# wonheeML/mtl-ssl

Hardware: AMD Instinct MI355X
Metric: images/sec training, Faster R-CNN ResNet-101 + aux heads (higher is better)
Workload: dtype f32; 1 GPU; Faster R-CNN ResNet-101 + window/closeness/edgemask heads + refine, synthetic 1024x600 COCO-shaped (90 classes), per-GPU batch 2 (BASELINE.json configs[1]); global_batch=2, parallelism=dp1, pipeline_config=configs/frcnn_resnet101_coco_mtl.config

## Files before the change

### mtl_ssl_amd/csrc/conv.hip

```cpp
#include <stdlib.h>

#include <atomic>
#include <mutex>
#include <unordered_map>

#include "conv_mfma.h"
#include "conv_split.h"

namespace mtlssl {

__global__ void __launch_bounds__(256) k_row_group_flags(const float* __restrict__ scale, int n, uint8_t* __restrict__ flags) {
  const int i = blockIdx.x * blockDim.x + threadIdx.x;
  if (i < n) flags[i] = scale[i] != 0.f;
}
__global__ void __launch_bounds__(256) k_active_ksteps(const uint8_t* __restrict__ flags, int rpg, int P, int pps, int stride,
                                                       int* __restrict__ out) {
  const int z = blockIdx.x, pix0 = z * pps, pix1 = min(P, pix0 + pps);
  const int ksteps = (max(pix1 - pix0, 0) + BK - 1) / BK;
  const int lane = threadIdx.x & 63, w = threadIdx.x >> 6;
  int* list = out + KSTEP_HDR + (int64_t)z * stride;
  __shared__ int wave_cnt[4];
  int base = 0;
  for (int s0 = 0; s0 < ksteps; s0 += 256) {
    const int s = s0 + threadIdx.x;
// ... 1421 lines not shown
  MTLSSL_REQUIRE(!group_active || rows_per_group > 0, "conv_dgrad: group_active needs rows_per_group > 0");
  MTLSSL_REQUIRE(!(epi & MASK_ANY) || mask_ref, "conv_dgrad: mask_ref pointer required");
  MTLSSL_REQUIRE(!(epi & MTLSSL_EPI_RESIDUAL) || residual, "conv_dgrad: residual pointer required");
  ConvArgs p = make_args(d);
  p.a = dy; p.b = w; p.out = dx; p.residual = residual; p.mask = mask_ref; p.epi = epi;
  p.a_bytes = ydy_bytes(d);
  p.b_bytes = (unsigned)((int64_t)d->R * d->S * d->C * d->K * 4);
  p.M = d->N * d->H * d->W;
  p.NG = d->C;
  MTLSSL_REQUIRE(desc_dense(d) || mfma_dgrad_ok(d),
                 "conv_dgrad: a strided dy (ldy = %d) needs K %% 16 == 0, C %% 4 == 0 and C >= 16", d->ldy);
  const Route r = route(d, MODE_DGRAD, workspace != nullptr);
  switch (r.family) {
    case FAM_WINO:
      wino_dgrad(d, r.wc.variant, r.wc.tile, dy, w, residual, mask_ref, dx, epi, workspace, S(stream),
                 (filter_xf && xf_variant == r.wc.variant) ? filter_xf : nullptr);
      break;
    case FAM_PARITY:
      parity_dgrad(r, d, dy, w, residual, mask_ref, dx, epi, workspace, S(stream));
      break;
    case FAM_DIRECT:
      if (group_active && row_skip_ref().load() != 0 && desc_is_pointwise(d)) {
        p.group_active = group_active;
        p.rows_per_group = rows_per_group;
      }
      launch_planned<MODE_DGRAD>(r.plan, p, (float*)workspace, S(stream));
      break;
    case FAM_PADDED: {
      float* dy_pad = (float*)workspace;
      float* w_pad = (float*)((char*)workspace + r.front_a);
      hipLaunchKernelGGL(k_pad_rows, dim3(cdiv((int64_t)p.M * r.q.K, 256)), dim3(256), 0, S(stream), dy, (int64_t)p.M, d->K, r.q.K, dy_pad);
// ... 108 lines not shown
  if (int rc = check_desc(d)) return rc;
  static const int32_t PUBLIC[] = {MTLSSL_PLAN_WINO_F43, MTLSSL_PLAN_DIRECT, MTLSSL_PLAN_PARITY, MTLSSL_PLAN_PADDED, MTLSSL_PLAN_S2D,
                                   MTLSSL_PLAN_THIN,     MTLSSL_PLAN_VALU,   MTLSSL_PLAN_VALU,   MTLSSL_PLAN_VALU,   MTLSSL_PLAN_VALU};
  const Route r = route(d, mode);
  const mtlssl_conv_desc& q = r.q;
  for (int i = 0; i < MTLSSL_PLAN_INFO_LEN; ++i) out[i] = 0;
  out[0] = PUBLIC[r.family];
  out[1] = mtlssl_conv2d_tile_config(d, mode);
  out[2] = -1;
  out[14] = mtlssl_conv2d_num_dispatches(d, mode);
  const int64_t P = (int64_t)d->N * d->OH * d->OW, M = mode == MODE_FWD ? P : (int64_t)d->N * d->H * d->W;
  switch (r.family) {
    case FAM_WINO:
      if (r.wc.variant != 0) out[0] = MTLSSL_PLAN_WINO_M7;
      out[2] = r.wc.tile; out[3] = 1;
      out[9] = (int32_t)(mode == MODE_WGRAD ? d->C : M);
      out[10] = mode == MODE_DGRAD ? d->C : d->K;
      out[11] = CFG_BM[r.wc.tile]; out[12] = CFG_BN[r.wc.tile];
      break;
    case FAM_PARITY: {
      MTLSSL_REQUIRE(parity_class >= 0 && parity_class < 4, "plan_info: parity class %d of an input-parity dgrad", parity_class);
      const ParityProblem c = parity_problem(d, parity_class >> 1, parity_class & 1);
      if (c.Hs == 0 || c.Ws == 0 || c.Rs == 0 || c.Ss == 0) break;
      const Plan& pl = r.parity[parity_class];
      plan_info_gemm(pl, (int64_t)d->N * c.Hs * c.Ws, d->C, c.Rs * c.Ss * (d->K / CFG_BK[pl.cfg]), out);
      break;
    }
    case FAM_DIRECT: case FAM_PADDED: case FAM_S2D:
      if (mode == MODE_WGRAD) {
        const int cfg = r.wg.cfg;
// ... 103 lines not shown
  bool colsum_folded = false;
  auto colsum_partial = [&]() {
    const int kg = (int)cdiv(d->K, (d->K & 3) ? 1 : 4);
    dim3 grid(cdiv(kg, cp.CQ), cp.chunks);
    if (d->K & 3)
      hipLaunchKernelGGL(k_colsum_partial<float>, grid, dim3(256), 0, st, dy, (int)P, d->K, ldy, cp.per_chunk, cp.CQ,
                         (float*)workspace);
    else
      hipLaunchKernelGGL(k_colsum_partial<floatx4>, grid, dim3(256), 0, st, dy, (int)P, d->K, ldy, cp.per_chunk, cp.CQ,
                         (float*)workspace);
  };
  const Route r = route(d, MODE_WGRAD);
  switch (r.family) {
    case FAM_WINO:
      wino_wgrad(d, r.wc.variant, r.wc.tile, x, dy, out_scale, dw, beta, ws_main, st,
                 (input_xf && input_variant == r.wc.variant) ? input_xf : nullptr);
      break;
    case FAM_DIRECT: {
      const bool split = wgrad_on_split_engine(r, d);
      const int ns = split ? r.split_ns : r.wg.nsplit, pps = split ? r.split_pps : r.wg.pps;
      const bool ride = dbias && !split && ns <= COLSUM_MAX_PARTS;
      if (dbias && !ride) colsum_partial();
      p.out = ws_main;
      p.M = d->C; p.NG = d->K; p.nsplit = ns; p.pix_per_split = pps;
      p.cs_part = ride ? (float*)workspace : nullptr;
      if (group_active && row_skip_ref().load() != 0 && !split && desc_is_pointwise(d) && pointwise_ref().load() != 0 &&
          ns <= KSTEP_HDR) {
        int* list = (int*)((char*)ws_main + r.bytes);
        const int stride = (int)cdiv(pps, BK);
        hipLaunchKernelGGL(k_active_ksteps, dim3(ns), dim3(256), 0, st, group_active, rows_per_group, (int)P, pps, stride, list);
        p.k_steps = list;
// ... 60 lines not shown
```

### mtl_ssl_amd/csrc/conv_mfma.h

```cpp
#pragma once
#include <type_traits>

#include "common.h"

namespace mtlssl {

typedef float floatx16 __attribute__((ext_vector_type(16)));
typedef float floatx4 __attribute__((ext_vector_type(4)));

enum { MODE_FWD = 0, MODE_DGRAD = 1, MODE_WGRAD = 2 };
__device__ __forceinline__ float act_mask(float g, float y, int epi) {
  bool on = y > 0.f && (!(epi & MTLSSL_EPI_MASK6) || y < 6.f);
  return on ? g : 0.f;
}
constexpr int MASK_ANY = MTLSSL_EPI_MASK | MTLSSL_EPI_MASK6;
constexpr int BK = 16;
#ifndef MTLSSL_LAB_FLAGS
#define MTLSSL_LAB_FLAGS 0
#endif
constexpr int LAB = MTLSSL_LAB_FLAGS;

struct ConvArgs {
  const float* a;
  const float* b;
// ... 184 lines not shown
  constexpr bool B_KC = (MODE == MODE_DGRAD);
  constexpr int A_LD = BM / RP, B_LD = BN / RP;
  constexpr unsigned OOB = 0xFFFFFFF0u;
  constexpr int LDT = 36;
  constexpr int SMEM_OPS = 2 * BKT * (LDA + LDB), SMEM_EPI = NW * 32 * LDT;
  __shared__ __attribute__((aligned(16))) float smem[SMEM_OPS > SMEM_EPI ? SMEM_OPS : SMEM_EPI];
  float* const sA = smem;
  float* const sB = smem + 2 * BKT * LDA;

  int nwg = p.tiles_m * p.tiles_n;
  int bid = blockIdx.x;
  {
    int q = nwg / 8, r = nwg % 8, xcd = bid % 8, loc = bid / 8;
    bid = (xcd < r ? xcd * (q + 1) : r * (q + 1) + (xcd - r) * q) + loc;
  }
  const int tile_m = bid / p.tiles_n + p.tile_m0, tile_n = bid % p.tiles_n;
  const int m0 = tile_m * BM, n0 = tile_n * BN;
  const int tid = threadIdx.x, lane = tid & 63, wid = tid >> 6;
  const int wr = wid >> 1, wc = wid & 1;
  const int lo = lane & 31, hi = lane >> 5;
  const int kq4 = (tid % KQ) * 4;

  if constexpr (BATCH) {
    p.a += (int64_t)blockIdx.y * p.a_bs;
    p.b += (int64_t)blockIdx.y * p.b_bs;
    if constexpr (MODE != MODE_WGRAD) p.out += (int64_t)blockIdx.y * p.o_bs;
  }
  if constexpr (MODE == MODE_WGRAD && !BATCH) {
    if (p.a_tab) {
      const int grp = blockIdx.z / p.nsplit;
// ... 3 lines not shown
  }
  const int ldy = args_ldy(p);
  int rs_fixed = 0, pix0 = 0, pix1 = 0, ksteps, ks_begin = 0;
  const int* steps = nullptr;
  if constexpr (MODE == MODE_FWD) {
    ksteps = p.R * p.S * (p.C / BKT);
  } else if constexpr (MODE == MODE_DGRAD) {
    ksteps = p.R * p.S * (p.K / BKT);
  } else {
    rs_fixed = BATCH ? 0 : blockIdx.y;
    int split = (!BATCH && p.a_tab) ? blockIdx.z % p.nsplit : blockIdx.z;
    int P = p.N * p.OH * p.OW;
    pix0 = split * p.pix_per_split;
    pix1 = min(P, pix0 + p.pix_per_split);
    ksteps = (max(pix1 - pix0, 0) + BKT - 1) / BKT;
    if constexpr (PW && !BATCH)
      if (p.k_steps) {
        steps = p.k_steps + KSTEP_HDR + split * p.k_stride;
        ksteps = p.k_steps[split];
      }
  }
  unsigned a_rec = p.a_bytes, b_rec = p.b_bytes;
  if constexpr (PW && MODE == MODE_WGRAD) {
    a_rec = min(a_rec, (unsigned)(max(pix1, 0) * p.C) * 4u);
    b_rec = min(b_rec, (unsigned)(max(pix1, 0) * ldy) * 4u);
  }
  __amdgpu_buffer_rsrc_t rsrc_a = __builtin_amdgcn_make_buffer_rsrc(const_cast<float*>(p.a), 0, a_rec, 0x00020000);
  __amdgpu_buffer_rsrc_t rsrc_b = __builtin_amdgcn_make_buffer_rsrc(const_cast<float*>(p.b), 0, b_rec, 0x00020000);
  if constexpr (MODE != MODE_WGRAD) {
    if (p.nsplit > 1) {
      ks_begin = blockIdx.z * p.ks_per_split;
      ksteps = min(ksteps, ks_begin + p.ks_per_split);
    }
  }
  if constexpr (PW && MODE == MODE_DGRAD && !SEG && !BATCH)
    if (p.group_active && !tile_rows_active(p, m0, BM)) ksteps = ks_begin;

  int a_base[A_LD], a_y[A_LD], a_x[A_LD], a_n[A_LD];
  bool a_ok[A_LD];
  unsigned a_voff[A_LD];
  unsigned b_base[B_LD];
  if constexpr (PW && MODE == MODE_WGRAD) {
#pragma unroll
    for (int i = 0; i < A_LD; ++i) {
      const int u = tid + NT * i;
      const int col = m0 + (u % (BM / 4)) * 4;
      a_voff[i] = col < p.M ? (unsigned)((pix0 + u / (BM / 4)) * p.C + col) * 4u : OOB;
    }
  } else if constexpr (PW) {
#pragma unroll
    for (int i = 0; i < A_LD; ++i) {
// ... 348 lines not shown
  constexpr int STAGE = A_FL + B_FL;
  constexpr int PA = BM * BKT / 256 / NW, PB = BN * BKT / 256 / NW;
  constexpr int G = BKT / 8;
  constexpr unsigned OOB = 0xFFFFFFF0u;
  constexpr int LDT = 36;
  constexpr int SMEM_OPS = NSTAGE * STAGE, SMEM_EPI = NW * 32 * LDT;
  __shared__ __attribute__((aligned(16))) float smem[SMEM_OPS > SMEM_EPI ? SMEM_OPS : SMEM_EPI];
  typedef __attribute__((address_space(3))) void* lds_ptr_t;

  int nwg = p.tiles_m * p.tiles_n;
  int bid = blockIdx.x;
  {
    int q = nwg / 8, r = nwg % 8, xcd = bid % 8, loc = bid / 8;
    bid = (xcd < r ? xcd * (q + 1) : r * (q + 1) + (xcd - r) * q) + loc;
  }
  const int tile_m = bid / p.tiles_n + p.tile_m0, tile_n = bid % p.tiles_n;
  const int m0 = tile_m * BM, n0 = tile_n * BN;
  const int tid = threadIdx.x, lane = tid & 63, wid = tid >> 6;
  const int wr = wid >> 1, wc = wid & 1;
  const int lo = lane & 31, hi = lane >> 5;
  auto kc_row = [&](int piece) { return piece * RPP + lane / QPR; };
  auto kc_quad4 = [&](int row) { return (((lane % QPR) ^ ((row >> RSH) & (QPR - 1)))) * 4; };

  if constexpr (BATCH) {
    p.a += (int64_t)blockIdx.y * p.a_bs;
    p.b += (int64_t)blockIdx.y * p.b_bs;
    if constexpr (MODE != MODE_WGRAD) p.out += (int64_t)blockIdx.y * p.o_bs;
  }
  int rs_fixed = 0, pix0 = 0, pix1 = 0, ksteps, ks_begin = 0;
  const int* steps = nullptr;
  if constexpr (MODE == MODE_FWD) {
    ksteps = p.R * p.S * (p.C / BKT);
  } else if constexpr (MODE == MODE_DGRAD) {
    ksteps = p.R * p.S * (p.K / BKT);
  } else {
    rs_fixed = BATCH ? 0 : blockIdx.y;
    int split = blockIdx.z;
    int P = p.N * p.OH * p.OW;
    pix0 = split * p.pix_per_split;
    pix1 = min(P, pix0 + p.pix_per_split);
    ksteps = (max(pix1 - pix0, 0) + BKT - 1) / BKT;
    if constexpr (PWISE && !BATCH)
      if (p.k_steps) {
        steps = p.k_steps + KSTEP_HDR + split * p.k_stride;
        ksteps = p.k_steps[split];
      }
  }
  if constexpr (MODE != MODE_WGRAD) {
    if (p.nsplit > 1) {
      ks_begin = blockIdx.z * p.ks_per_split;
      ksteps = min(ksteps, ks_begin + p.ks_per_split);
    }
  }
  if constexpr (PWISE && MODE == MODE_DGRAD && !BATCH)
    if (p.group_active && !tile_rows_active(p, m0, BM)) ksteps = ks_begin;

  const int ldy = args_ldy(p);
  unsigned a_rec = p.a_bytes, b_rec = p.b_bytes;
  if constexpr (PWISE && MODE == MODE_WGRAD) {
    a_rec = min(a_rec, (unsigned)(max(pix1, 0) * p.C) * 4u);
    b_rec = min(b_rec, (unsigned)(max(pix1, 0) * ldy) * 4u);
  }
  const __amdgpu_buffer_rsrc_t rsrc_a = __builtin_amdgcn_make_buffer_rsrc(const_cast<float*>(p.a), 0, a_rec, 0x00020000);
  const __amdgpu_buffer_rsrc_t rsrc_b = __builtin_amdgcn_make_buffer_rsrc(const_cast<float*>(p.b), 0, b_rec, 0x00020000);

  int a_base[PA], a_y[PA], a_x[PA], a_n[PA], a_q4[PA];
  bool a_ok[PA];
  unsigned a_voff[PA];
  unsigned b_base[PB];
  if constexpr (PWISE && MODE == MODE_WGRAD) {
// ... 381 lines not shown
  double occ_eff = occ <= 1 ? 0.55 : (occ == 2 ? 0.80 : 1.0);
  double step_us = CFG_BM[cfg] * CFG_BN[cfg] * 2.0 * CFG_BK[cfg] / 614e9 * 1e6 / (base_eff[cfg & 3] * occ_eff);
  return (double)per_cu * (ksteps_per_block + 96 / CFG_BK[cfg]) * step_us;
}

enum { WINO_F43 = 0, WINO_M7 = 1, WINO_VARIANTS = 2 };
bool wino_eligible(const mtlssl_conv_desc* d, int variant);
double wino_time_us(const mtlssl_conv_desc* d, int variant, int mode, int* tile);
int64_t wino_workspace_bytes(const mtlssl_conv_desc* d, int variant, int mode);
void wino_fwd(const mtlssl_conv_desc* d, int variant, int tile, const float* x, const float* w, const float* bias,
              const float* residual, float* y, int epi, void* workspace, hipStream_t st, const float* filter_xf = nullptr,
              float* input_xf_keep = nullptr);
int64_t wino_input_bytes(const mtlssl_conv_desc* d, int variant);
void wino_dgrad(const mtlssl_conv_desc* d, int variant, int tile, const float* dy, const float* w,
                const float* residual, const float* mask_ref, float* dx, int epi, void* workspace, hipStream_t st,
                const float* filter_xf = nullptr);
int64_t wino_filter_bytes(const mtlssl_conv_desc* d, int variant);
void wino_filter(const mtlssl_conv_desc* d, int variant, int flip, const float* w, float* U, hipStream_t st);
void wino_filters_batched(int variant, int n, const void* w_ptrs, const void* u_ptrs, const int64_t* ck,
                          const int32_t* flip, int64_t max_ck, hipStream_t st);
void wino_wgrad(const mtlssl_conv_desc* d, int variant, int tile, const float* x, const float* dy,
                const float* out_scale, float* dw, float beta, void* workspace, hipStream_t st,
                const float* input_xf = nullptr);

}
```

### mtl_ssl_amd/csrc/winograd.hip

```cpp
#include "conv_mfma.h"
#include "conv_split.h"

namespace mtlssl {

namespace {

struct F43 {
  static constexpr int P = 6, I = 6, O = 4;
  static constexpr float bt(int a, int i) {
    constexpr float t[6][6] = {{4, 0, -5, 0, 1, 0}, {0, -4, -4, 1, 1, 0}, {0, 4, -4, -1, 1, 0},
                               {0, -2, -1, 2, 1, 0}, {0, 2, -1, -2, 1, 0}, {0, 4, 0, -5, 0, 1}};
    return t[a][i];
  }
  static constexpr float at(int u, int a) {
    constexpr float t[4][6] = {{1, 1, 1, 1, 1, 0}, {0, 1, -1, 2, -2, 0}, {0, 1, 1, 4, 4, 0}, {0, 1, -1, 8, -8, 1}};
    return t[u][a];
  }
  static constexpr float g(int a, int r) {
    constexpr float t[6][3] = {{1.f / 4, 0, 0}, {-1.f / 6, -1.f / 6, -1.f / 6}, {-1.f / 6, 1.f / 6, -1.f / 6},
                               {1.f / 24, 1.f / 12, 1.f / 6}, {1.f / 24, -1.f / 12, 1.f / 6}, {0, 0, 1}};
    return t[a][r];
  }
};
struct F33 {
// ... 41 lines not shown
        if (first) acc = (c == 1.f) ? d[i] : c * d[i];
        else if (c == 1.f) acc = acc + d[i];
        else if (c == -1.f) acc = acc - d[i];
        else acc = acc + c * d[i];
        first = false;
      }
    }
    o[a] = acc;
  }
}

struct WinoGeom {
  int N, H, W, th, tw;
  int64_t T;
};
struct TileIdx { int64_t t; int c, n, ty, tx; bool ok; };
template <typename VT>
__device__ __forceinline__ TileIdx tile_index(const WinoGeom& g, int C) {
  constexpr int VW = sizeof(VT) / 4;
  TileIdx r;
  const int cq = C / VW;
  int64_t idx = blockIdx.x * (int64_t)256 + threadIdx.x;
  r.ok = idx < g.T * cq;
  r.c = (int)(idx % cq) * VW;
  r.t = idx / cq;
  r.tx = (int)(r.t % g.tw);
  int64_t q = r.t / g.tw;
  r.ty = (int)(q % g.th);
  r.n = (int)(q / g.th);
  return r;
}
__device__ __forceinline__ float act_fwd(float v, int epi) {
  if (epi & MTLSSL_EPI_RELU) v = fmaxf(v, 0.f);
  if (epi & MTLSSL_EPI_RELU6) v = fminf(fmaxf(v, 0.f), 6.f);
  if (epi & MTLSSL_EPI_TANH) v = tanhf(v);
  return v;
}
__device__ __forceinline__ floatx4 act_fwd(floatx4 v, int epi) {
#pragma unroll
  for (int q = 0; q < 4; ++q) v[q] = act_fwd(v[q], epi);
  return v;
}
// ... 33 lines not shown
  int64_t i = (blockIdx.x * (int64_t)256 + threadIdx.x) * (sizeof(VT) / 4);
  if (i >= CK) return;
  wino_filter_one<S, VT>(w, U, CK, flip, i);
}
template <typename S>
__global__ void __launch_bounds__(256) k_wino_filter_batched(const float* const* w, float* const* U, const int64_t* CK,
                                                             const int32_t* flip) {
  const int l = blockIdx.y;
  const int64_t ck = CK[l];
  int64_t i = blockIdx.x * (int64_t)256 + threadIdx.x;
  if (i >= ck) return;
  wino_filter_one<S, float>(w[l], U[l], ck, flip[l], i);
}

template <typename S, typename VT>
__global__ void __launch_bounds__(256) k_wino_input(const float* in, float* V, WinoGeom g, int C, int ld) {
  constexpr int P = S::P, I = S::I;
  const TileIdx ix = tile_index<VT>(g, C);
  if (!ix.ok) return;
  const int y0 = S::O * ix.ty - 1, x0 = S::O * ix.tx - 1;
  const float* base = in + ((int64_t)ix.n * g.H * g.W) * ld + ix.c;
  VT tmp[P][I];
#pragma unroll
  for (int j = 0; j < I; ++j) {
    const int x = x0 + j;
    const bool okx = (unsigned)x < (unsigned)g.W;
    VT col[I], o[P];
#pragma unroll
    for (int i = 0; i < I; ++i) {
      const int y = y0 + i;
      const bool ok = okx && (unsigned)y < (unsigned)g.H;
      col[i] = ok ? *reinterpret_cast<const VT*>(base + ((int64_t)y * g.W + x) * ld) : VT{};
    }
    xform<S, XF_BT, P, I>(col, o);
#pragma unroll
    for (int a = 0; a < P; ++a) tmp[a][j] = o[a];
  }
  const int64_t plane = g.T * C;
  float* vp = V + ix.t * C + ix.c;
#pragma unroll
  for (int a = 0; a < P; ++a) {
    VT o[P];
    xform<S, XF_BT, P, I>(tmp[a], o);
#pragma unroll
    for (int b = 0; b < P; ++b) *reinterpret_cast<VT*>(vp + (int64_t)(a * P + b) * plane) = o[b];
  }
}

template <typename S, typename VT>
__global__ void __launch_bounds__(256) k_wino_dy(const float* dy, float* dM, WinoGeom g, int K, int ld) {
  constexpr int P = S::P, O = S::O;
  const TileIdx ix = tile_index<VT>(g, K);
  if (!ix.ok) return;
  const float* base = dy + ((int64_t)ix.n * g.H * g.W) * ld + ix.c;
  VT tmp[P][O];
#pragma unroll
  for (int j = 0; j < O; ++j) {
    const int x = O * ix.tx + j;
    VT col[O], o[P];
#pragma unroll
    for (int i = 0; i < O; ++i) {
      const int y = O * ix.ty + i;
      const bool ok = y < g.H && x < g.W;
      col[i] = ok ? *reinterpret_cast<const VT*>(base + ((int64_t)y * g.W + x) * ld) : VT{};
    }
    xform<S, XF_A, P, O>(col, o);
#pragma unroll
    for (int a = 0; a < P; ++a) tmp[a][j] = o[a];
  }
  const int64_t plane = g.T * K;
  float* mp = dM + ix.t * K + ix.c;
#pragma unroll
  for (int a = 0; a < P; ++a) {
    VT o[P];
    xform<S, XF_A, P, O>(tmp[a], o);
#pragma unroll
    for (int b = 0; b < P; ++b) *reinterpret_cast<VT*>(mp + (int64_t)(a * P + b) * plane) = o[b];
  }
}

template <typename S, int MODE, typename VT>
__global__ void __launch_bounds__(256) k_wino_output(const float* Mb, float* out, WinoGeom g, int K, int ldo,
                                                     const float* bias, const float* residual,
                                                     const float* mask, int epi) {
  constexpr int P = S::P, O = S::O;
  const TileIdx ix = tile_index<VT>(g, K);
  if (!ix.ok) return;
  const int64_t plane = g.T * K;
  const float* mp = Mb + ix.t * K + ix.c;
  VT tmp[O][P];
#pragma unroll
  for (int b = 0; b < P; ++b) {
    VT col[P], o[O];
#pragma unroll
    for (int a = 0; a < P; ++a) col[a] = *reinterpret_cast<const VT*>(mp + (int64_t)(a * P + b) * plane);
    xform<S, XF_AT, O, P>(col, o);
#pragma unroll
    for (int u = 0; u < O; ++u) tmp[u][b] = o[u];
  }
  VT bv{};
  if constexpr (MODE == MODE_FWD)
    if (epi & MTLSSL_EPI_BIAS) bv = *reinterpret_cast<const VT*>(bias + ix.c);
#pragma unroll
  for (int u = 0; u < O; ++u) {
    VT o[O];
    xform<S, XF_AT, O, P>(tmp[u], o);
    const int oy = O * ix.ty + u;
    if (oy >= g.H) continue;
#pragma unroll
    for (int v_ = 0; v_ < O; ++v_) {
// ... 48 lines not shown
  VT sc{};
  if (scale) sc = *reinterpret_cast<const VT*>(scale + i % K);
#pragma unroll
  for (int r = 0; r < 3; ++r) {
    VT o[3];
    xform<S, XF_GT, 3, P>(t[r], o);
#pragma unroll
    for (int s = 0; s < 3; ++s) {
      VT v = scale ? o[s] * sc : o[s];
      VT* p = reinterpret_cast<VT*>(dw + (int64_t)(r * 3 + s) * CK + i);
      *p = beta != 0.f ? beta * *p + v : v;
    }
  }
}

typedef float floatx2 __attribute__((ext_vector_type(2)));

template <typename S>
WinoGeom geom(const mtlssl_conv_desc* d) {
  WinoGeom g;
  g.N = d->N; g.H = d->H; g.W = d->W;
  g.th = (int)cdiv(d->H, S::O); g.tw = (int)cdiv(d->W, S::O);
  g.T = (int64_t)d->N * g.th * g.tw;
  return g;
}

template <typename S> constexpr bool can_vec() { return S::P <= 6; }
inline bool wide(int64_t T, int C) { return T * C / 4 >= 131072; }

template <typename S>
void run_filter(const float* w, float* U, int64_t CK, int flip, hipStream_t st) {
  if constexpr (can_vec<S>()) {
    if (CK >= 262144) {
      hipLaunchKernelGGL((k_wino_filter<S, floatx4>), dim3(cdiv(CK / 4, 256)), dim3(256), 0, st, w, U, CK, flip);
      return;
    }
  }
  hipLaunchKernelGGL((k_wino_filter<S, float>), dim3(cdiv(CK, 256)), dim3(256), 0, st, w, U, CK, flip);
}
template <typename S>
void run_input(const float* in, float* V, const WinoGeom& g, int C, hipStream_t st, int ld = 0) {
  if (ld <= 0) ld = C;
  if constexpr (can_vec<S>()) {
    if (wide(g.T, C)) {
      hipLaunchKernelGGL((k_wino_input<S, floatx4>), dim3(cdiv(g.T * C / 4, 256)), dim3(256), 0, st, in, V, g, C, ld);
      return;
    }
  }
  hipLaunchKernelGGL((k_wino_input<S, float>), dim3(cdiv(g.T * C, 256)), dim3(256), 0, st, in, V, g, C, ld);
}
template <typename S>
void run_dy(const float* dy, float* dM, const WinoGeom& g, int K, hipStream_t st, int ld = 0) {
  if (ld <= 0) ld = K;
  if constexpr (can_vec<S>()) {
    if (wide(g.T, K)) {
      hipLaunchKernelGGL((k_wino_dy<S, floatx4>), dim3(cdiv(g.T * K / 4, 256)), dim3(256), 0, st, dy, dM, g, K, ld);
      return;
    }
  }
  hipLaunchKernelGGL((k_wino_dy<S, float>), dim3(cdiv(g.T * K, 256)), dim3(256), 0, st, dy, dM, g, K, ld);
}
template <typename S, int MODE>
void run_output(const float* Mb, float* out, const WinoGeom& g, int K, const float* bias, const float* residual,
                const float* mask, int epi, hipStream_t st, int ldo = 0) {
  if (ldo <= 0) ldo = K;
  if constexpr (can_vec<S>()) {
    if (wide(g.T, K)) {
      hipLaunchKernelGGL((k_wino_output<S, MODE, floatx4>), dim3(cdiv(g.T * K / 4, 256)), dim3(256), 0, st, Mb, out,
                         g, K, ldo, bias, residual, mask, epi);
      return;
    }
  }
  hipLaunchKernelGGL((k_wino_output<S, MODE, float>), dim3(cdiv(g.T * K, 256)), dim3(256), 0, st, Mb, out, g, K, ldo,
                     bias, residual, mask, epi);
}
template <typename S>
void run_wgrad_out(const float* dU, int ns, int64_t CK, int K, const float* scale, float* dw, float beta,
                   hipStream_t st) {
  if constexpr (can_vec<S>()) {
    if (CK >= 262144) {
      hipLaunchKernelGGL((k_wino_wgrad_out<S, floatx2>), dim3(cdiv(CK / 2, 256)), dim3(256), 0, st, dU, ns, CK, K,
                         scale, dw, beta);
      return;
    }
  }
  hipLaunchKernelGGL((k_wino_wgrad_out<S, float>), dim3(cdiv(CK, 256)), dim3(256), 0, st, dU, ns, CK, K, scale, dw,
                     beta);
}

// ... 78 lines not shown
  if (mode == MODE_WGRAD) {
    cfg = best_tile(d->C, d->K, PL, (int)cdiv(g.T, 16), &tg);
    int ns, pps;
    wgrad_split(g.T, PL, d->C, d->K, cfg, &ns, &pps);
    tg = tile_time_us(cfg, cdiv(d->C, CFG_BM[cfg]) * cdiv(d->K, CFG_BN[cfg]) * PL * ns, pps / 16, true);
    bytes = 4.0 * (px * (d->C + d->K) + 2.0 * PL * g.T * (d->C + d->K) + (double)PL * d->C * d->K * (ns + 1));
  } else {
    int cin = mode == MODE_FWD ? d->C : d->K, cout = mode == MODE_FWD ? d->K : d->C;
    cfg = best_tile(g.T, cout, PL, cin / 16, &tg);
    bytes = 4.0 * (px * (cin + cout) + 2.0 * PL * g.T * (cin + cout) + 2.0 * PL * d->C * d->K);
  }
  if (tile) *tile = cfg;
  return tg + bytes / 4.0e6 + 12.0;
}

template <typename S>
int64_t workspace_bytes(const mtlssl_conv_desc* d, int mode) {
  constexpr int PL = S::P * S::P;
  WinoGeom g = geom<S>(d);
  int64_t planes = align_up((int64_t)PL * g.T * d->C * 4, 256) + align_up((int64_t)PL * g.T * d->K * 4, 256);
  if (mode == MODE_WGRAD) {
    int ns = 1, pps;
    int64_t mx = 1;
    for (int cfg = 0; cfg < NCFG; ++cfg) { wgrad_split(g.T, PL, d->C, d->K, cfg, &ns, &pps); if (ns > mx) mx = ns; }
    if (split_wgrad_plan(g.T, d->C, d->K, PL, &ns, &pps) && ns > mx) mx = ns;
    return planes + align_up(mx * PL * d->C * d->K * 4, 256);
  }
  return planes + align_up((int64_t)PL * d->C * d->K * 4, 256);
}

template <typename S>
void fwd(const mtlssl_conv_desc* d, int tile, const float* x, const float* w, const float* bias,
         const float* residual, float* y, int epi, void* workspace, hipStream_t st, const float* U_pre = nullptr,
         float* V_keep = nullptr) {
  constexpr int PL = S::P * S::P;
// ... 5 lines not shown
  if (U_pre) U = const_cast<float*>(U_pre);
  else run_filter<S>(w, U, CK, 0, st);
  if (V_keep) V = V_keep;
  run_input<S>(x, V, g, d->C, st);
  ConvArgs p = gemm_args(g.T, d->C, d->K);
  p.a = V; p.b = U; p.out = Mb;
  p.M = (int)g.T; p.NG = d->K;
  p.a_bytes = (unsigned)(g.T * d->C * 4); p.b_bytes = (unsigned)(CK * 4);
  p.a_bs = g.T * d->C; p.b_bs = CK; p.o_bs = g.T * d->K;
  launch_gemm<MODE_FWD>(tile, p, PL, 1, st);
  run_output<S, MODE_FWD>(Mb, y, g, d->K, bias, residual, nullptr, epi, st, d->ldy);
}

template <typename S>
void dgrad(const mtlssl_conv_desc* d, int tile, const float* dy, const float* w, const float* residual,
           const float* mask_ref, float* dx, int epi, void* workspace, hipStream_t st, const float* U_pre = nullptr) {
  constexpr int PL = S::P * S::P;
  WinoGeom g = geom<S>(d);
  const int64_t CK = (int64_t)d->C * d->K;
  float* U = (float*)workspace;
  float* V = (float*)((char*)U + align_up(PL * CK * 4, 256));
  float* Mb = (float*)((char*)V + align_up((int64_t)PL * g.T * d->K * 4, 256));
  if (U_pre) U = const_cast<float*>(U_pre);
  else run_filter<S>(w, U, CK, 1, st);
  run_input<S>(dy, V, g, d->K, st, d->ldy);
  ConvArgs p = gemm_args(g.T, d->C, d->K);
  p.a = V; p.b = U; p.out = Mb;
  p.M = (int)g.T; p.NG = d->C;
  p.a_bytes = (unsigned)(g.T * d->K * 4); p.b_bytes = (unsigned)(CK * 4);
  p.a_bs = g.T * d->K; p.b_bs = CK; p.o_bs = g.T * d->C;
  launch_gemm<MODE_DGRAD>(tile, p, PL, 1, st);
  run_output<S, MODE_DGRAD>(Mb, dx, g, d->C, nullptr, residual, mask_ref, epi, st);
}

template <typename S>
void wgrad(const mtlssl_conv_desc* d, int tile, const float* x, const float* dy, const float* out_scale,
           float* dw, float beta, void* workspace, hipStream_t st, const float* V_pre = nullptr) {
  constexpr int PL = S::P * S::P;
  WinoGeom g = geom<S>(d);
  const int64_t CK = (int64_t)d->C * d->K;
  float* V = (float*)workspace;
  float* dM = (float*)((char*)V + align_up((int64_t)PL * g.T * d->C * 4, 256));
  float* dU = (float*)((char*)dM + align_up((int64_t)PL * g.T * d->K * 4, 256));
  int ns, pps;
  wgrad_split(g.T, PL, d->C, d->K, tile, &ns, &pps);
  const bool split = fp32_engine() >= 1 && (tile == 0 || tile == 3) && split_wgrad_plan(g.T, d->C, d->K, PL, &ns, &pps);
  if (V_pre) V = const_cast<float*>(V_pre);
  else run_input<S>(x, V, g, d->C, st);
  run_dy<S>(dy, dM, g, d->K, st, d->ldy);
  ConvArgs p = gemm_args(g.T, d->C, d->K);
  p.a = V; p.b = dM; p.out = dU;
  p.M = d->C; p.NG = d->K; p.nsplit = ns; p.pix_per_split = pps;
  p.a_bytes = (unsigned)(g.T * d->C * 4); p.b_bytes = (unsigned)(g.T * d->K * 4);
  p.a_bs = g.T * d->C; p.b_bs = g.T * d->K;
  if (split) launch_split<MODE_WGRAD, true>(p, dim3(1, PL, ns), st);
  else launch_gemm<MODE_WGRAD>(tile, p, PL, ns, st);
  run_wgrad_out<S>(dU, ns, CK, d->K, out_scale, dw, beta, st);
}

}

bool wino_eligible(const mtlssl_conv_desc* d, int variant) {
  return variant == WINO_M7 ? eligible<M7>(d) : eligible<F43>(d);
}
double wino_time_us(const mtlssl_conv_desc* d, int variant, int mode, int* tile) {
// ... 3 lines not shown
  return variant == WINO_M7 ? workspace_bytes<M7>(d, mode) : workspace_bytes<F43>(d, mode);
}
void wino_fwd(const mtlssl_conv_desc* d, int variant, int tile, const float* x, const float* w, const float* bias,
              const float* residual, float* y, int epi, void* workspace, hipStream_t st, const float* filter_xf,
              float* input_xf_keep) {
  if (variant == WINO_M7) fwd<M7>(d, tile, x, w, bias, residual, y, epi, workspace, st, filter_xf, input_xf_keep);
  else fwd<F43>(d, tile, x, w, bias, residual, y, epi, workspace, st, filter_xf, input_xf_keep);
}
int64_t wino_input_bytes(const mtlssl_conv_desc* d, int variant) {
  if (variant == WINO_M7) { WinoGeom g = geom<M7>(d); return align_up((int64_t)M7::P * M7::P * g.T * d->C * 4, 256); }
  WinoGeom g = geom<F43>(d);
  return align_up((int64_t)F43::P * F43::P * g.T * d->C * 4, 256);
}
void wino_dgrad(const mtlssl_conv_desc* d, int variant, int tile, const float* dy, const float* w,
                const float* residual, const float* mask_ref, float* dx, int epi, void* workspace, hipStream_t st,
                const float* filter_xf) {
  if (variant == WINO_M7) dgrad<M7>(d, tile, dy, w, residual, mask_ref, dx, epi, workspace, st, filter_xf);
  else dgrad<F43>(d, tile, dy, w, residual, mask_ref, dx, epi, workspace, st, filter_xf);
}
int64_t wino_filter_bytes(const mtlssl_conv_desc* d, int variant) {
  const int64_t pl = variant == WINO_M7 ? M7::P * M7::P : F43::P * F43::P;
  return align_up(pl * (int64_t)d->C * d->K * 4, 256);
}
void wino_filters_batched(int variant, int n, const void* w_ptrs, const void* u_ptrs, const int64_t* ck,
                          const int32_t* flip, int64_t max_ck, hipStream_t st) {
  dim3 grid((unsigned)cdiv(max_ck, 256), n);
  if (variant == WINO_M7)
    hipLaunchKernelGGL((k_wino_filter_batched<M7>), grid, dim3(256), 0, st, (const float* const*)w_ptrs,
                       (float* const*)u_ptrs, ck, flip);
  else
    hipLaunchKernelGGL((k_wino_filter_batched<F43>), grid, dim3(256), 0, st, (const float* const*)w_ptrs,
                       (float* const*)u_ptrs, ck, flip);
}
void wino_filter(const mtlssl_conv_desc* d, int variant, int flip, const float* w, float* U, hipStream_t st) {
  const int64_t CK = (int64_t)d->C * d->K;
  if (variant == WINO_M7) run_filter<M7>(w, U, CK, flip, st);
  else run_filter<F43>(w, U, CK, flip, st);
}
void wino_wgrad(const mtlssl_conv_desc* d, int variant, int tile, const float* x, const float* dy,
                const float* out_scale, float* dw, float beta, void* workspace, hipStream_t st, const float* input_xf) {
  if (variant == WINO_M7) wgrad<M7>(d, tile, x, dy, out_scale, dw, beta, workspace, st, input_xf);
  else wgrad<F43>(d, tile, x, dy, out_scale, dw, beta, workspace, st, input_xf);
}

}
```

### mtl_ssl_amd/nn.py

```python
import torch

from . import ops

f32 = torch.float32


def _refresh_bn(layer):
    if layer.bn_trainable:
        ps = layer.ps
        if layer.gamma is not None:
            torch.mul(ps.value(layer.gamma.name), layer.inv_std, out=layer.scale)
        torch.addcmul(ps.value(layer.beta.name), ps.value(layer.mean.name), layer.scale, value=-1.0,
                      out=layer.shift)


class WgradStream:

    def __init__(self, stream):
        self.stream = stream

    def run(self, layer, x, g, **kw):
        if not layer.trainable:
            return
        ev = torch.cuda.Event()
# ... 305 lines not shown

    def backward(self, gp, ctx, need_input_grad=True, mask_input=True, wgrad=INLINE_WGRAD, active=None):
        kw = {} if active is None else dict(active=active)
        x, a1, a2, sc_sub = ctx[:4]
        if self.bn_trainable:
            out, sc = ctx[4], ctx[5]
            o3 = ops.axpby(sc, out.clone(), -1.0, 1.0)
            self.conv3.bn_grad(o3, gp)
            del o3
            if self.shortcut is not None:
                self.shortcut.bn_grad(sc, gp)
        wgrad.run(self.conv3, a2, gp, **kw)
        gp2 = self.conv3.dgrad(a2.shape, gp, mask_ref=a2, **kw)
        if self.bn_trainable:
            self.conv2.bn_grad(a2, gp2)
        wgrad.run(self.conv2, a1, gp2)
        gp1 = self.conv2.dgrad(a1.shape, gp2, mask_ref=a1)
        if self.bn_trainable:
            self.conv1.bn_grad(a1, gp1)
        wgrad.run(self.conv1, x, gp1, **kw)
        if self.shortcut is not None:
            wgrad.run(self.shortcut, x, gp, **kw)
        if not need_input_grad:
            return None
        if self.shortcut is not None:
            addend = self.shortcut.dgrad(x.shape, gp, **kw)
        elif self.stride > 1:
            addend = ops.maxpool_bwd(x, sc_sub, gp, 1, self.stride, (0, 0))
        else:
            addend = gp
        return self.conv1.dgrad(x.shape, gp1, residual=addend, mask_ref=x if mask_input else None, **kw)

# ... 70 lines not shown
```

Before: 40.57 images/sec.

## Skip inactive batch images in Winograd dgrad and wgrad via compacted tile maps

Extends the per-image activity (row-skip) mechanism to the Winograd 3x3 conv path used by the bottleneck middle conv. For dgrad it compacts active tiles into a dense slot map so the transform, batched GEMM and output only touch live images, and whole GEMM workgroups exit early. For wgrad it builds per-split compacted k-step lists so the GEMM reduces only over active tiles. This adds index-building kernels, extra workspace and a gather copy when a pre-transformed input is reused, and only pays off when some images in the batch are inactive.

```diff
diff --git a/mtl_ssl_amd/csrc/conv.hip b/mtl_ssl_amd/csrc/conv.hip
--- a/mtl_ssl_amd/csrc/conv.hip
+++ b/mtl_ssl_amd/csrc/conv.hip
@@ -1459,7 +1459,8 @@
   switch (r.family) {
     case FAM_WINO:
       wino_dgrad(d, r.wc.variant, r.wc.tile, dy, w, residual, mask_ref, dx, epi, workspace, S(stream),
-                 (filter_xf && xf_variant == r.wc.variant) ? filter_xf : nullptr);
+                 (filter_xf && xf_variant == r.wc.variant) ? filter_xf : nullptr,
+                 (group_active && row_skip_ref().load() != 0 && rows_per_group == d->H * d->W) ? group_active : nullptr);
       break;
     case FAM_PARITY:
       parity_dgrad(r, d, dy, w, residual, mask_ref, dx, epi, workspace, S(stream));
@@ -1598,6 +1599,12 @@
     case FAM_WINO:
       if (r.wc.variant != 0) out[0] = MTLSSL_PLAN_WINO_M7;
       out[2] = r.wc.tile; out[3] = 1;
+      if (mode == MODE_WGRAD) {
+        int ns, pps;
+        wino_wgrad_split(d, r.wc.variant, r.wc.tile, &ns, &pps);
+        const int64_t T = wino_input_bytes(d, r.wc.variant) / ((r.wc.variant != 0 ? 121 : 36) * 4 * (int64_t)d->C);
+        out[3] = ns; out[4] = pps / BK; out[8] = (int32_t)cdiv(T, BK); out[13] = pps;
+      }
       out[9] = (int32_t)(mode == MODE_WGRAD ? d->C : M);
       out[10] = mode == MODE_DGRAD ? d->C : d->K;
       out[11] = CFG_BM[r.wc.tile]; out[12] = CFG_BN[r.wc.tile];
@@ -1731,7 +1738,8 @@
   switch (r.family) {
     case FAM_WINO:
       wino_wgrad(d, r.wc.variant, r.wc.tile, x, dy, out_scale, dw, beta, ws_main, st,
-                 (input_xf && input_variant == r.wc.variant) ? input_xf : nullptr);
+                 (input_xf && input_variant == r.wc.variant) ? input_xf : nullptr,
+                 (group_active && row_skip_ref().load() != 0 && rows_per_group == d->OH * d->OW) ? group_active : nullptr);
       break;
     case FAM_DIRECT: {
       const bool split = wgrad_on_split_engine(r, d);
diff --git a/mtl_ssl_amd/csrc/conv_mfma.h b/mtl_ssl_amd/csrc/conv_mfma.h
--- a/mtl_ssl_amd/csrc/conv_mfma.h
+++ b/mtl_ssl_amd/csrc/conv_mfma.h
@@ -222,6 +222,8 @@
     int q = nwg / 8, r = nwg % 8, xcd = bid % 8, loc = bid / 8;
     bid = (xcd < r ? xcd * (q + 1) : r * (q + 1) + (xcd - r) * q) + loc;
   }
+  if constexpr (BATCH && MODE == MODE_DGRAD)
+    if (p.group_active) bid = (int)((bid + (unsigned)blockIdx.y * ((nwg + 7) / 8)) % (unsigned)nwg);
   const int tile_m = bid / p.tiles_n + p.tile_m0, tile_n = bid % p.tiles_n;
   const int m0 = tile_m * BM, n0 = tile_n * BN;
   const int tid = threadIdx.x, lane = tid & 63, wid = tid >> 6;
@@ -255,7 +257,7 @@
     pix0 = split * p.pix_per_split;
     pix1 = min(P, pix0 + p.pix_per_split);
     ksteps = (max(pix1 - pix0, 0) + BKT - 1) / BKT;
-    if constexpr (PW && !BATCH)
+    if constexpr (PW)
       if (p.k_steps) {
         steps = p.k_steps + KSTEP_HDR + split * p.k_stride;
         ksteps = p.k_steps[split];
@@ -274,8 +276,11 @@
       ksteps = min(ksteps, ks_begin + p.ks_per_split);
     }
   }
-  if constexpr (PW && MODE == MODE_DGRAD && !SEG && !BATCH)
-    if (p.group_active && !tile_rows_active(p, m0, BM)) ksteps = ks_begin;
+  if constexpr (PW && MODE == MODE_DGRAD && !SEG)
+    if (p.group_active && !tile_rows_active(p, m0, BM)) {
+      if constexpr (BATCH) return;
+      ksteps = ks_begin;
+    }
 
   int a_base[A_LD], a_y[A_LD], a_x[A_LD], a_n[A_LD];
   bool a_ok[A_LD];
@@ -654,6 +659,8 @@
     int q = nwg / 8, r = nwg % 8, xcd = bid % 8, loc = bid / 8;
     bid = (xcd < r ? xcd * (q + 1) : r * (q + 1) + (xcd - r) * q) + loc;
   }
+  if constexpr (BATCH && MODE == MODE_DGRAD)
+    if (p.group_active) bid = (int)((bid + (unsigned)blockIdx.y * ((nwg + 7) / 8)) % (unsigned)nwg);
   const int tile_m = bid / p.tiles_n + p.tile_m0, tile_n = bid % p.tiles_n;
   const int m0 = tile_m * BM, n0 = tile_n * BN;
   const int tid = threadIdx.x, lane = tid & 63, wid = tid >> 6;
@@ -680,7 +687,7 @@
     pix0 = split * p.pix_per_split;
     pix1 = min(P, pix0 + p.pix_per_split);
     ksteps = (max(pix1 - pix0, 0) + BKT - 1) / BKT;
-    if constexpr (PWISE && !BATCH)
+    if constexpr (PWISE)
       if (p.k_steps) {
         steps = p.k_steps + KSTEP_HDR + split * p.k_stride;
         ksteps = p.k_steps[split];
@@ -692,8 +699,11 @@
       ksteps = min(ksteps, ks_begin + p.ks_per_split);
     }
   }
-  if constexpr (PWISE && MODE == MODE_DGRAD && !BATCH)
-    if (p.group_active && !tile_rows_active(p, m0, BM)) ksteps = ks_begin;
+  if constexpr (PWISE && MODE == MODE_DGRAD)
+    if (p.group_active && !tile_rows_active(p, m0, BM)) {
+      if constexpr (BATCH) return;
+      ksteps = ks_begin;
+    }
 
   const int ldy = args_ldy(p);
   unsigned a_rec = p.a_bytes, b_rec = p.b_bytes;
@@ -1105,13 +1115,14 @@
 int64_t wino_input_bytes(const mtlssl_conv_desc* d, int variant);
 void wino_dgrad(const mtlssl_conv_desc* d, int variant, int tile, const float* dy, const float* w,
                 const float* residual, const float* mask_ref, float* dx, int epi, void* workspace, hipStream_t st,
-                const float* filter_xf = nullptr);
+                const float* filter_xf = nullptr, const uint8_t* batch_active = nullptr);
 int64_t wino_filter_bytes(const mtlssl_conv_desc* d, int variant);
 void wino_filter(const mtlssl_conv_desc* d, int variant, int flip, const float* w, float* U, hipStream_t st);
 void wino_filters_batched(int variant, int n, const void* w_ptrs, const void* u_ptrs, const int64_t* ck,
                           const int32_t* flip, int64_t max_ck, hipStream_t st);
 void wino_wgrad(const mtlssl_conv_desc* d, int variant, int tile, const float* x, const float* dy,
                 const float* out_scale, float* dw, float beta, void* workspace, hipStream_t st,
-                const float* input_xf = nullptr);
-
-}
+                const float* input_xf = nullptr, const uint8_t* batch_active = nullptr);
+void wino_wgrad_split(const mtlssl_conv_desc* d, int variant, int tile, int* ns, int* pps);
+
+}
diff --git a/mtl_ssl_amd/csrc/winograd.hip b/mtl_ssl_amd/csrc/winograd.hip
--- a/mtl_ssl_amd/csrc/winograd.hip
+++ b/mtl_ssl_amd/csrc/winograd.hip
@@ -79,9 +79,10 @@
   int N, H, W, th, tw;
   int64_t T;
 };
-struct TileIdx { int64_t t; int c, n, ty, tx; bool ok; };
+constexpr int ROW_ZERO = -1, ROW_SKIP = -2;
+struct TileIdx { int64_t t; int c, n, ty, tx; bool ok, zero; };
 template <typename VT>
-__device__ __forceinline__ TileIdx tile_index(const WinoGeom& g, int C) {
+__device__ __forceinline__ TileIdx tile_index(const WinoGeom& g, int C, const int* row_src = nullptr) {
   constexpr int VW = sizeof(VT) / 4;
   TileIdx r;
   const int cq = C / VW;
@@ -89,8 +90,16 @@
   r.ok = idx < g.T * cq;
   r.c = (int)(idx % cq) * VW;
   r.t = idx / cq;
-  r.tx = (int)(r.t % g.tw);
-  int64_t q = r.t / g.tw;
+  r.zero = false;
+  int64_t src = r.t;
+  if (row_src && r.ok) {
+    const int m = row_src[r.t];
+    r.ok = m != ROW_SKIP;
+    r.zero = m == ROW_ZERO;
+    src = m < 0 ? 0 : m;
+  }
+  r.tx = (int)(src % g.tw);
+  int64_t q = src / g.tw;
   r.ty = (int)(q % g.th);
   r.n = (int)(q / g.th);
   return r;
@@ -154,9 +163,10 @@
 }
 
 template <typename S, typename VT>
-__global__ void __launch_bounds__(256) k_wino_input(const float* in, float* V, WinoGeom g, int C, int ld) {
+__global__ void __launch_bounds__(256) k_wino_input(const float* in, float* V, WinoGeom g, int C, int ld,
+                                                    const int* row_src) {
   constexpr int P = S::P, I = S::I;
-  const TileIdx ix = tile_index<VT>(g, C);
+  const TileIdx ix = tile_index<VT>(g, C, row_src);
   if (!ix.ok) return;
   const int y0 = S::O * ix.ty - 1, x0 = S::O * ix.tx - 1;
   const float* base = in + ((int64_t)ix.n * g.H * g.W) * ld + ix.c;
@@ -164,7 +174,7 @@
 #pragma unroll
   for (int j = 0; j < I; ++j) {
     const int x = x0 + j;
-    const bool okx = (unsigned)x < (unsigned)g.W;
+    const bool okx = (unsigned)x < (unsigned)g.W && !ix.zero;
     VT col[I], o[P];
 #pragma unroll
     for (int i = 0; i < I; ++i) {
@@ -188,9 +198,10 @@
 }
 
 template <typename S, typename VT>
-__global__ void __launch_bounds__(256) k_wino_dy(const float* dy, float* dM, WinoGeom g, int K, int ld) {
+__global__ void __launch_bounds__(256) k_wino_dy(const float* dy, float* dM, WinoGeom g, int K, int ld,
+                                                 const int* row_src) {
   constexpr int P = S::P, O = S::O;
-  const TileIdx ix = tile_index<VT>(g, K);
+  const TileIdx ix = tile_index<VT>(g, K, row_src);
   if (!ix.ok) return;
   const float* base = dy + ((int64_t)ix.n * g.H * g.W) * ld + ix.c;
   VT tmp[P][O];
@@ -201,7 +212,7 @@
 #pragma unroll
     for (int i = 0; i < O; ++i) {
       const int y = O * ix.ty + i;
-      const bool ok = y < g.H && x < g.W;
+      const bool ok = y < g.H && x < g.W && !ix.zero;
       col[i] = ok ? *reinterpret_cast<const VT*>(base + ((int64_t)y * g.W + x) * ld) : VT{};
     }
     xform<S, XF_A, P, O>(col, o);
@@ -222,18 +233,20 @@
 template <typename S, int MODE, typename VT>
 __global__ void __launch_bounds__(256) k_wino_output(const float* Mb, float* out, WinoGeom g, int K, int ldo,
                                                      const float* bias, const float* residual,
-                                                     const float* mask, int epi) {
+                                                     const float* mask, int epi, const int* slot) {
   constexpr int P = S::P, O = S::O;
   const TileIdx ix = tile_index<VT>(g, K);
   if (!ix.ok) return;
   const int64_t plane = g.T * K;
-  const float* mp = Mb + ix.t * K + ix.c;
+  const int row = slot ? slot[ix.t] : 0;
+  const bool live = row >= 0;
+  const float* mp = Mb + (slot ? (int64_t)(live ? row : 0) : ix.t) * K + ix.c;
   VT tmp[O][P];
 #pragma unroll
   for (int b = 0; b < P; ++b) {
     VT col[P], o[O];
 #pragma unroll
-    for (int a = 0; a < P; ++a) col[a] = *reinterpret_cast<const VT*>(mp + (int64_t)(a * P + b) * plane);
+    for (int a = 0; a < P; ++a) col[a] = live ? *reinterpret_cast<const VT*>(mp + (int64_t)(a * P + b) * plane) : VT{};
     xform<S, XF_AT, O, P>(col, o);
 #pragma unroll
     for (int u = 0; u < O; ++u) tmp[u][b] = o[u];
@@ -312,6 +325,80 @@
   }
 }
 
+__global__ void __launch_bounds__(256) k_wino_active_tiles(const uint8_t* __restrict__ flags, int tpg, int T,
+                                                           int* __restrict__ slot, int* __restrict__ row_src,
+                                                           uint8_t* __restrict__ gflags) {
+  const int lane = threadIdx.x & 63, w = threadIdx.x >> 6;
+  __shared__ int wave_cnt[4];
+  int base = 0;
+  for (int t0 = 0; t0 < T; t0 += 256) {
+    const int t = t0 + threadIdx.x;
+    const bool act = t < T && flags[t / tpg] != 0;
+    const unsigned long long m = __ballot(act);
+    if (lane == 0) wave_cnt[w] = __popcll(m);
+    __syncthreads();
+    int off = base;
+    for (int i = 0; i < w; ++i) off += wave_cnt[i];
+    const int row = off + __popcll(m & ((1ull << lane) - 1ull));
+    if (t < T) slot[t] = act ? row : -1;
+    if (act) row_src[row] = t;
+    base += wave_cnt[0] + wave_cnt[1] + wave_cnt[2] + wave_cnt[3];
+    __syncthreads();
+  }
+  for (int r = base + threadIdx.x; r < T; r += 256) row_src[r] = ROW_SKIP;
+  for (int i = threadIdx.x; i < (T + 63) / 64; i += 256) gflags[i] = i * 64 < base;
+}
+__global__ void __launch_bounds__(256) k_wino_active_pairs(const uint8_t* __restrict__ flags, int tpg, int T, int pps, int glds,
+                                                           int stride, int* __restrict__ row_src, int* __restrict__ out) {
+  const int z = blockIdx.x, pix0 = z * pps, pix1 = min(T, pix0 + pps);
+  const int npairs = (max(pix1 - pix0, 0) + BK - 1) / BK * (BK / 2);
+  const int lane = threadIdx.x & 63, w = threadIdx.x >> 6;
+  auto row_of = [&](int q, int h) { return pix0 + BK * (q >> 3) + (glds ? (q & 7) + 8 * h : 2 * (q & 7) + h); };
+  auto live = [&](int r) { return r < pix1 && flags[r / tpg] != 0; };
+  __shared__ int wave_cnt[4];
+  int base = 0;
+  for (int q0 = 0; q0 < npairs; q0 += 256) {
+    const int q = q0 + threadIdx.x;
+    const bool act = q < npairs && (live(row_of(q, 0)) || live(row_of(q, 1)));
+    const unsigned long long m = __ballot(act);
+    if (lane == 0) wave_cnt[w] = __popcll(m);
+    __syncthreads();
+    int off = base;
+    for (int i = 0; i < w; ++i) off += wave_cnt[i];
+    if (act) {
+      const int j = off + __popcll(m & ((1ull << lane) - 1ull));
+      for (int h = 0; h < 2; ++h) {
+        const int dst = row_of(j, h), src = row_of(q, h);
+        if (dst < pix1) row_src[dst] = src < pix1 ? src : ROW_ZERO;
+      }
+    }
+    base += wave_cnt[0] + wave_cnt[1] + wave_cnt[2] + wave_cnt[3];
+    __syncthreads();
+  }
+  const int ksteps = (base + 7) / 8;
+  for (int j = base + threadIdx.x; j < npairs; j += 256)
+    for (int h = 0; h < 2; ++h) {
+      const int dst = row_of(j, h);
+      if (dst < pix1) row_src[dst] = j < ksteps * 8 ? ROW_ZERO : ROW_SKIP;
+    }
+  if (threadIdx.x == 0) out[z] = ksteps;
+  for (int i = threadIdx.x; i < ksteps; i += 256) out[KSTEP_HDR + (int64_t)z * stride + i] = i;
+}
+__global__ void __launch_bounds__(256) k_wino_gather_rows(const float* __restrict__ src, float* __restrict__ dst,
+                                                          const int* __restrict__ row_src, int64_t T, int C) {
+  const int cq = C / 4;
+  const int64_t idx = blockIdx.x * (int64_t)256 + threadIdx.x;
+  if (idx >= T * cq) return;
+  const int64_t r = idx / cq;
+  const int c = (int)(idx % cq) * 4;
+  const int m = row_src[r];
+  if (m == ROW_SKIP) return;
+  const int64_t plane = (int64_t)blockIdx.y * T * C;
+  floatx4 v = {0.f, 0.f, 0.f, 0.f};
+  if (m >= 0) v = *reinterpret_cast<const floatx4*>(src + plane + (int64_t)m * C + c);
+  *reinterpret_cast<floatx4*>(dst + plane + r * C + c) = v;
+}
+
 typedef float floatx2 __attribute__((ext_vector_type(2)));
 
 template <typename S>
@@ -337,40 +424,44 @@
   hipLaunchKernelGGL((k_wino_filter<S, float>), dim3(cdiv(CK, 256)), dim3(256), 0, st, w, U, CK, flip);
 }
 template <typename S>
-void run_input(const float* in, float* V, const WinoGeom& g, int C, hipStream_t st, int ld = 0) {
+void run_input(const float* in, float* V, const WinoGeom& g, int C, hipStream_t st, int ld = 0,
+               const int* row_src = nullptr) {
   if (ld <= 0) ld = C;
   if constexpr (can_vec<S>()) {
     if (wide(g.T, C)) {
-      hipLaunchKernelGGL((k_wino_input<S, floatx4>), dim3(cdiv(g.T * C / 4, 256)), dim3(256), 0, st, in, V, g, C, ld);
+      hipLaunchKernelGGL((k_wino_input<S, floatx4>), dim3(cdiv(g.T * C / 4, 256)), dim3(256), 0, st, in, V, g, C, ld,
+                         row_src);
       return;
     }
   }
-  hipLaunchKernelGGL((k_wino_input<S, float>), dim3(cdiv(g.T * C, 256)), dim3(256), 0, st, in, V, g, C, ld);
-}
-template <typename S>
-void run_dy(const float* dy, float* dM, const WinoGeom& g, int K, hipStream_t st, int ld = 0) {
+  hipLaunchKernelGGL((k_wino_input<S, float>), dim3(cdiv(g.T * C, 256)), dim3(256), 0, st, in, V, g, C, ld, row_src);
+}
+template <typename S>
+void run_dy(const float* dy, float* dM, const WinoGeom& g, int K, hipStream_t st, int ld = 0,
+            const int* row_src = nullptr) {
   if (ld <= 0) ld = K;
   if constexpr (can_vec<S>()) {
     if (wide(g.T, K)) {
-      hipLaunchKernelGGL((k_wino_dy<S, floatx4>), dim3(cdiv(g.T * K / 4, 256)), dim3(256), 0, st, dy, dM, g, K, ld);
+      hipLaunchKernelGGL((k_wino_dy<S, floatx4>), dim3(cdiv(g.T * K / 4, 256)), dim3(256), 0, st, dy, dM, g, K, ld,
+                         row_src);
       return;
     }
   }
-  hipLaunchKernelGGL((k_wino_dy<S, float>), dim3(cdiv(g.T * K, 256)), dim3(256), 0, st, dy, dM, g, K, ld);
+  hipLaunchKernelGGL((k_wino_dy<S, float>), dim3(cdiv(g.T * K, 256)), dim3(256), 0, st, dy, dM, g, K, ld, row_src);
 }
 template <typename S, int MODE>
 void run_output(const float* Mb, float* out, const WinoGeom& g, int K, const float* bias, const float* residual,
-                const float* mask, int epi, hipStream_t st, int ldo = 0) {
+                const float* mask, int epi, hipStream_t st, int ldo = 0, const int* slot = nullptr) {
   if (ldo <= 0) ldo = K;
   if constexpr (can_vec<S>()) {
     if (wide(g.T, K)) {
       hipLaunchKernelGGL((k_wino_output<S, MODE, floatx4>), dim3(cdiv(g.T * K / 4, 256)), dim3(256), 0, st, Mb, out,
-                         g, K, ldo, bias, residual, mask, epi);
+                         g, K, ldo, bias, residual, mask, epi, slot);
       return;
     }
   }
   hipLaunchKernelGGL((k_wino_output<S, MODE, float>), dim3(cdiv(g.T * K, 256)), dim3(256), 0, st, Mb, out, g, K, ldo,
-                     bias, residual, mask, epi);
+                     bias, residual, mask, epi, slot);
 }
 template <typename S>
 void run_wgrad_out(const float* dU, int ns, int64_t CK, int K, const float* scale, float* dw, float beta,
@@ -479,11 +570,16 @@
   return tg + bytes / 4.0e6 + 12.0;
 }
 
+inline int64_t index_bytes(int64_t T) {
+  const int64_t Tp = align_up(T, 64);
+  return align_up((2 * Tp + KSTEP_HDR + Tp / 16 + 16) * 4 + Tp / 64, 256);
+}
 template <typename S>
 int64_t workspace_bytes(const mtlssl_conv_desc* d, int mode) {
   constexpr int PL = S::P * S::P;
   WinoGeom g = geom<S>(d);
   int64_t planes = align_up((int64_t)PL * g.T * d->C * 4, 256) + align_up((int64_t)PL * g.T * d->K * 4, 256);
+  if (mode != MODE_FWD) planes += index_bytes(g.T);
   if (mode == MODE_WGRAD) {
     int ns = 1, pps;
     int64_t mx = 1;
@@ -519,7 +615,8 @@
 
 template <typename S>
 void dgrad(const mtlssl_conv_desc* d, int tile, const float* dy, const float* w, const float* residual,
-           const float* mask_ref, float* dx, int epi, void* workspace, hipStream_t st, const float* U_pre = nullptr) {
+           const float* mask_ref, float* dx, int epi, void* workspace, hipStream_t st, const float* U_pre = nullptr,
+           const uint8_t* active = nullptr) {
   constexpr int PL = S::P * S::P;
   WinoGeom g = geom<S>(d);
   const int64_t CK = (int64_t)d->C * d->K;
@@ -528,19 +625,30 @@
   float* Mb = (float*)((char*)V + align_up((int64_t)PL * g.T * d->K * 4, 256));
   if (U_pre) U = const_cast<float*>(U_pre);
   else run_filter<S>(w, U, CK, 1, st);
-  run_input<S>(dy, V, g, d->K, st, d->ldy);
   ConvArgs p = gemm_args(g.T, d->C, d->K);
   p.a = V; p.b = U; p.out = Mb;
   p.M = (int)g.T; p.NG = d->C;
   p.a_bytes = (unsigned)(g.T * d->K * 4); p.b_bytes = (unsigned)(CK * 4);
   p.a_bs = g.T * d->K; p.b_bs = CK; p.o_bs = g.T * d->C;
+  const int* slot = nullptr;
+  const int* row_src = nullptr;
+  if (active && !split_engine_takes(tile, p.M, p.NG, p.C, PL)) {
+    const int64_t Tp = align_up(g.T, 64);
+    int* maps = (int*)((char*)workspace + workspace_bytes<S>(d, MODE_DGRAD) - index_bytes(g.T));
+    uint8_t* gflags = (uint8_t*)(maps + 2 * Tp);
+    hipLaunchKernelGGL(k_wino_active_tiles, dim3(1), dim3(256), 0, st, active, g.th * g.tw, (int)g.T, maps, maps + Tp, gflags);
+    slot = maps; row_src = maps + Tp;
+    p.group_active = gflags; p.rows_per_group = 64;
+  }
+  run_input<S>(dy, V, g, d->K, st, d->ldy, row_src);
   launch_gemm<MODE_DGRAD>(tile, p, PL, 1, st);
-  run_output<S, MODE_DGRAD>(Mb, dx, g, d->C, nullptr, residual, mask_ref, epi, st);
+  run_output<S, MODE_DGRAD>(Mb, dx, g, d->C, nullptr, residual, mask_ref, epi, st, 0, slot);
 }
 
 template <typename S>
 void wgrad(const mtlssl_conv_desc* d, int tile, const float* x, const float* dy, const float* out_scale,
-           float* dw, float beta, void* workspace, hipStream_t st, const float* V_pre = nullptr) {
+           float* dw, float beta, void* workspace, hipStream_t st, const float* V_pre = nullptr,
+           const uint8_t* active = nullptr) {
   constexpr int PL = S::P * S::P;
   WinoGeom g = geom<S>(d);
   const int64_t CK = (int64_t)d->C * d->K;
@@ -550,10 +658,21 @@
   int ns, pps;
   wgrad_split(g.T, PL, d->C, d->K, tile, &ns, &pps);
   const bool split = fp32_engine() >= 1 && (tile == 0 || tile == 3) && split_wgrad_plan(g.T, d->C, d->K, PL, &ns, &pps);
-  if (V_pre) V = const_cast<float*>(V_pre);
-  else run_input<S>(x, V, g, d->C, st);
-  run_dy<S>(dy, dM, g, d->K, st, d->ldy);
   ConvArgs p = gemm_args(g.T, d->C, d->K);
+  const int* row_src = nullptr;
+  if (active && !split && ns <= KSTEP_HDR) {
+    int* maps = (int*)((char*)workspace + workspace_bytes<S>(d, MODE_WGRAD) - index_bytes(g.T));
+    int* list = maps + align_up(g.T, 64);
+    hipLaunchKernelGGL(k_wino_active_pairs, dim3(ns), dim3(256), 0, st, active, g.th * g.tw, (int)g.T, pps,
+                       tile >= NCFG ? 1 : 0, pps / BK, maps, list);
+    row_src = maps;
+    p.k_steps = list; p.k_stride = pps / BK;
+  }
+  if (V_pre && row_src)
+    hipLaunchKernelGGL(k_wino_gather_rows, dim3(cdiv(g.T * d->C / 4, 256), PL), dim3(256), 0, st, V_pre, V, row_src, g.T, d->C);
+  else if (V_pre) V = const_cast<float*>(V_pre);
+  else run_input<S>(x, V, g, d->C, st, 0, row_src);
+  run_dy<S>(dy, dM, g, d->K, st, d->ldy, row_src);
   p.a = V; p.b = dM; p.out = dU;
   p.M = d->C; p.NG = d->K; p.nsplit = ns; p.pix_per_split = pps;
   p.a_bytes = (unsigned)(g.T * d->C * 4); p.b_bytes = (unsigned)(g.T * d->K * 4);
@@ -587,9 +706,9 @@
 }
 void wino_dgrad(const mtlssl_conv_desc* d, int variant, int tile, const float* dy, const float* w,
                 const float* residual, const float* mask_ref, float* dx, int epi, void* workspace, hipStream_t st,
-                const float* filter_xf) {
-  if (variant == WINO_M7) dgrad<M7>(d, tile, dy, w, residual, mask_ref, dx, epi, workspace, st, filter_xf);
-  else dgrad<F43>(d, tile, dy, w, residual, mask_ref, dx, epi, workspace, st, filter_xf);
+                const float* filter_xf, const uint8_t* batch_active) {
+  if (variant == WINO_M7) dgrad<M7>(d, tile, dy, w, residual, mask_ref, dx, epi, workspace, st, filter_xf, batch_active);
+  else dgrad<F43>(d, tile, dy, w, residual, mask_ref, dx, epi, workspace, st, filter_xf, batch_active);
 }
 int64_t wino_filter_bytes(const mtlssl_conv_desc* d, int variant) {
   const int64_t pl = variant == WINO_M7 ? M7::P * M7::P : F43::P * F43::P;
@@ -611,9 +730,16 @@
   else run_filter<F43>(w, U, CK, flip, st);
 }
 void wino_wgrad(const mtlssl_conv_desc* d, int variant, int tile, const float* x, const float* dy,
-                const float* out_scale, float* dw, float beta, void* workspace, hipStream_t st, const float* input_xf) {
-  if (variant == WINO_M7) wgrad<M7>(d, tile, x, dy, out_scale, dw, beta, workspace, st, input_xf);
-  else wgrad<F43>(d, tile, x, dy, out_scale, dw, beta, workspace, st, input_xf);
-}
-
-}
+                const float* out_scale, float* dw, float beta, void* workspace, hipStream_t st, const float* input_xf,
+                const uint8_t* batch_active) {
+  if (variant == WINO_M7) wgrad<M7>(d, tile, x, dy, out_scale, dw, beta, workspace, st, input_xf, batch_active);
+  else wgrad<F43>(d, tile, x, dy, out_scale, dw, beta, workspace, st, input_xf, batch_active);
+}
+void wino_wgrad_split(const mtlssl_conv_desc* d, int variant, int tile, int* ns, int* pps) {
+  const int PL = variant == WINO_M7 ? M7::P * M7::P : F43::P * F43::P;
+  const int64_t T = variant == WINO_M7 ? geom<M7>(d).T : geom<F43>(d).T;
+  wgrad_split(T, PL, d->C, d->K, tile, ns, pps);
+  if (fp32_engine() >= 1 && (tile == 0 || tile == 3)) split_wgrad_plan(T, d->C, d->K, PL, ns, pps);
+}
+
+}
diff --git a/mtl_ssl_amd/nn.py b/mtl_ssl_amd/nn.py
--- a/mtl_ssl_amd/nn.py
+++ b/mtl_ssl_amd/nn.py
@@ -343,8 +343,8 @@
         gp2 = self.conv3.dgrad(a2.shape, gp, mask_ref=a2, **kw)
         if self.bn_trainable:
             self.conv2.bn_grad(a2, gp2)
-        wgrad.run(self.conv2, a1, gp2)
-        gp1 = self.conv2.dgrad(a1.shape, gp2, mask_ref=a1)
+        wgrad.run(self.conv2, a1, gp2, **kw)
+        gp1 = self.conv2.dgrad(a1.shape, gp2, mask_ref=a1, **kw)
         if self.bn_trainable:
             self.conv1.bn_grad(a1, gp1)
         wgrad.run(self.conv1, x, gp1, **kw)
```

Measured after the change: 41.49 images/sec (median of 6 runs). +2.3%, better.
